# Crispy13/GeneFuseRust

Hardware: AMD Instinct MI355X
Metric: 150bp_reads_per_s_map_read_vs_druggable_shaped_index (higher is better)
Workload: dtype u32

## Files before the change

genefuserust_amd/csrc/gf_pipe_kernels.h:

```cpp
#pragma once

#include <hip/hip_runtime.h>

#include "../../include/gfmatch.h"
#include "gf_map_kernels.h"
#include "gf_table.h"

#ifndef GF_PROBE_NT
#define GF_PROBE_NT false
#endif

__device__ __forceinline__ uint32_t gf_spread16(uint32_t x) {
  x &= 0xFFFFu;
  x = (x | (x << 8)) & 0x00FF00FFu;
  x = (x | (x << 4)) & 0x0F0F0F0Fu;
  x = (x | (x << 2)) & 0x33333333u;
  x = (x | (x << 1)) & 0x55555555u;
  return x;
}

__device__ __forceinline__ uint32_t gf_gather_nibble_lsb(uint32_t x) {
  x &= 0x11111111u;
  x = (x | (x >> 3)) & 0x03030303u;
  x = (x | (x >> 6)) & 0x000F000Fu;
  x = (x | (x >> 12)) & 0xFFu;
  return x;
}

__device__ __forceinline__ unsigned int gf_wave_append(bool want, unsigned int* counter) {
  const uint64_t m = __ballot(want);
  unsigned int base = 0;
  if (m) {
    const int leader = __builtin_ctzll(m);
    if ((int)(threadIdx.x & 63) == leader) base = atomicAdd(counter, (unsigned int)__popcll(m));
    base = (unsigned int)__builtin_amdgcn_readlane((int)base, leader);
  }
  return base + (unsigned int)gf_lanes_below(m);
}

__device__ __forceinline__ unsigned int gf_wave_append_lds(bool want, unsigned int* s_counter) {
  const uint64_t m = __ballot(want);
  unsigned int base = 0;
  if (m) {
    const int leader = __builtin_ctzll(m);
    if ((int)(threadIdx.x & 63) == leader) base = atomicAdd(s_counter, (unsigned int)__popcll(m));
    base = (unsigned int)__builtin_amdgcn_readlane((int)base, leader);
  }
  return base + (unsigned int)gf_lanes_below(m);
}

#define GF_ENTRY_FILTERED 0x80000000u

template <int PW>
struct GfPipeEntryW {
  static constexpr int NT = PW <= 16 ? 4 : (PW + 3) / 4;
  static constexpr int EW = (2 + NT + PW + 3) / 4;
  uint32_t w[4 * EW];
};

template <int PW>
__device__ __forceinline__ void gf_entry_load(const GfPipeEntryW<PW>* e, uint32_t& r, uint32_t& v1v2,
                                              uint32_t (&m)[GfPipeEntryW<PW>::NT], uint32_t (&pk)[PW + 1]) {
  constexpr int NT = GfPipeEntryW<PW>::NT, EW = GfPipeEntryW<PW>::EW;
  uint32_t w[4 * EW];
  const gf_u32x4* src = (const gf_u32x4*)e;
#pragma unroll
  for (int j = 0; j < EW; ++j) {
#ifdef GF_ENTRY_NT
    const gf_u32x4 q = __builtin_nontemporal_load(src + j);
#else
    const gf_u32x4 q = src[j];
#endif
    w[4 * j] = q.x; w[4 * j + 1] = q.y; w[4 * j + 2] = q.z; w[4 * j + 3] = q.w;
  }
  r = w[0];
  v1v2 = w[1];
#pragma unroll
  for (int k = 0; k < NT; ++k) m[k] = w[2 + k];
#pragma unroll
  for (int j = 0; j < PW; ++j) pk[j] = w[2 + NT + j];
  pk[PW] = 0;
}

template <int PW>
__device__ __forceinline__ void gf_entry_store(GfPipeEntryW<PW>* e, uint32_t r, uint32_t v1v2,
                                               const uint32_t (&m)[GfPipeEntryW<PW>::NT], const uint32_t (&pk)[PW + 1]) {
  constexpr int NT = GfPipeEntryW<PW>::NT, EW = GfPipeEntryW<PW>::EW;
  uint32_t w[4 * EW];
  w[0] = r;
  w[1] = v1v2;
#pragma unroll
  for (int k = 0; k < NT; ++k) w[2 + k] = m[k];
#pragma unroll
  for (int j = 0; j < PW; ++j) w[2 + NT + j] = pk[j];
#pragma unroll
  for (int j = 2 + NT + PW; j < 4 * EW; ++j) w[j] = 0;
  gf_u32x4* dst = (gf_u32x4*)e;
#pragma unroll
  for (int j = 0; j < EW; ++j) {
    gf_u32x4 q;
    q.x = w[4 * j]; q.y = w[4 * j + 1]; q.z = w[4 * j + 2]; q.w = w[4 * j + 3];
#ifdef GF_ENTRY_NT
    __builtin_nontemporal_store(q, dst + j);
#else
    dst[j] = q;
#endif
  }
}

__device__ __forceinline__ uint32_t gf_cut_pk(const uint32_t* s_pk, uint32_t w0, uint32_t sh, int j) {
  return __builtin_amdgcn_alignbit(s_pk[w0 + j + 1], s_pk[w0 + j], sh);
}

__device__ __forceinline__ uint32_t gf_cut_iv(const uint32_t* s_iv, uint32_t pos, int L, int j) {
  const uint32_t bp = pos + 16u * (uint32_t)j;
  uint32_t b = __builtin_amdgcn_alignbit(s_iv[(bp >> 5) + 1], s_iv[bp >> 5], bp & 31u) & 0xFFFFu;
  const int k = L - 16 * j;
  if (k < 16) b |= k <= 0 ? 0xFFFFu : ((0xFFFFu << k) & 0xFFFFu);
  return gf_spread16(b);
}

__device__ __forceinline__ uint32_t gf_clean16(uint32_t z_lo, uint32_t z_hi) {
  uint32_t lo = ~z_lo & 0x55555555u, hi = ~z_hi & 0x55555555u;
#pragma unroll
  for (uint32_t sh = 2; sh <= 16; sh <<= 1) {
    lo &= __builtin_amdgcn_alignbit(hi, lo, sh);
    hi &= hi >> sh;
  }
  return lo;
}

__device__ __forceinline__ void gf_convert16(const uint4& q, uint32_t& code32, uint32_t& bad16) {
  const uint32_t z0 = q.x & 0x06060606u, z1 = q.y & 0x06060606u, z2 = q.z & 0x06060606u, z3 = q.w & 0x06060606u;
  const uint32_t d0 = q.x ^ __builtin_amdgcn_perm(0x00470054u, 0x00430041u, z0), d1 = q.y ^ __builtin_amdgcn_perm(0x00470054u, 0x00430041u, z1);
  const uint32_t d2 = q.z ^ __builtin_amdgcn_perm(0x00470054u, 0x00430041u, z2), d3 = q.w ^ __builtin_amdgcn_perm(0x00470054u, 0x00430041u, z3);
  const uint32_t e0 = __builtin_amdgcn_udot4(z0, 0x40100401u, 0u, false), e1 = __builtin_amdgcn_udot4(z1, 0x40100401u, 0u, false);
  const uint32_t e2 = __builtin_amdgcn_udot4(z2, 0x40100401u, 0u, false), e3 = __builtin_amdgcn_udot4(z3, 0x40100401u, 0u, false);
  code32 = ((e0 + (e1 << 8) + (e2 << 16)) >> 1) | ((e3 >> 1) << 24);
  bad16 = 0;
  if (d0 | d1 | d2 | d3) {
    const uint32_t n0 = (((d0 & 0x7F7F7F7Fu) + 0x7F7F7F7Fu) | d0) & 0x80808080u;
    const uint32_t n1 = (((d1 & 0x7F7F7F7Fu) + 0x7F7F7F7Fu) | d1) & 0x80808080u;
    const uint32_t n2 = (((d2 & 0x7F7F7F7Fu) + 0x7F7F7F7Fu) | d2) & 0x80808080u;
    const uint32_t n3 = (((d3 & 0x7F7F7F7Fu) + 0x7F7F7F7Fu) | d3) & 0x80808080u;
    bad16 = (((n0 >> 7) * 0x00204081u) >> 21 & 0xFu) | ((((n1 >> 7) * 0x00204081u) >> 21 & 0xFu) << 4) |
            ((((n2 >> 7) * 0x00204081u) >> 21 & 0xFu) << 8) | ((((n3 >> 7) * 0x00204081u) >> 21 & 0xFu) << 12);
  }
}

__device__ __forceinline__ uint32_t gf_window_mask(int nwin, int k) {
  const int m = nwin - 32 * k;
  return m >= 32 ? 0xFFFFFFFFu : (m <= 0 ? 0u : ((1u << m) - 1u));
}

#ifndef GF_SEED_FILTER_MASK
#define GF_SEED_FILTER_MASK 2u
#endif
#ifndef GF_MID_SEEDS
#define GF_MID_SEEDS 2
#endif
#ifndef GF_FILTER_AUX
#define GF_FILTER_AUX 0
#endif
#ifndef GF_SVS_WAVES_PER_SIMD
#define GF_SVS_WAVES_PER_SIMD 4
#endif
#ifndef GF_FQ_CAP
#define GF_FQ_CAP 96
#endif

template <int PW>
__device__ __forceinline__ int gf_filter_queue_pass(const GfTable& T, gf_u32x4* s_q, int q_len, int lane,
                                                    uint8_t* __restrict__ counts, GfPipeEntryW<PW>* my_list,
                                                    unsigned int* s_cnt) {
  static_assert(PW == 10, "the queue holds the 64-byte entries of reads of up to 160 bases");
  constexpr int NT = GfPipeEntryW<PW>::NT;
  const int m = q_len < 64 ? q_len : 64;
  const int base = q_len - m;
  const bool act = lane < m;
  uint32_t w[16];
#pragma unroll
  for (int j = 0; j < 16; ++j) w[j] = 0;
  if (act) {
#pragma unroll
    for (int j = 0; j < 4; ++j) {
      const gf_u32x4 q = s_q[(base + lane) * 4 + j];
      w[4 * j] = q.x; w[4 * j + 1] = q.y; w[4 * j + 2] = q.z; w[4 * j + 3] = q.w;
    }
  }
  gf_wave_lds_sync();
  const __amdgpu_buffer_rsrc_t filter_rsrc =
      __builtin_amdgcn_make_buffer_rsrc((void*)T.bloom, 0, (int)(T.bloom_words * 4u), 0x00020000);
  const uint32_t filter_bytes = T.bloom_words * 4u;
  const uint32_t rnd = w[1];
  bool alive = false;
  if (act) {
    uint32_t wlo = w[2 + NT];
#pragma unroll
    for (int j = 0; j < PW; ++j) {
      const uint32_t whi = j + 1 < PW ? w[2 + NT + j + 1] : 0u;
      const uint32_t byte = (w[2 + (j >> 2)] >> (8 * (j & 3))) & 0xFFu;
      uint32_t word[2], bits[2];
#pragma unroll
      for (int t = 0; t < 2; ++t) {
        const uint32_t s14 = __builtin_amdgcn_alignbit(whi, wlo, 16u * (uint32_t)t + 8u * rnd + 4u) & 0x0FFFFFFFu;
        const uint32_t h2 = GF_BLOOM_HASH((s14));
        bits[t] = GF_BLOOM_BITS(h2);
        const uint32_t nb = (byte & (3u << (4 * t + 2 * rnd))) ? filter_bytes : 0u;
        word[t] = __builtin_amdgcn_raw_buffer_load_b32(filter_rsrc, __umulhi(h2, nb) & ~3u, 0, GF_FILTER_AUX);
      }
      uint32_t fail2 = 0;
#pragma unroll
      for (int t = 0; t < 2; ++t) {
        const uint32_t d = bits[t] & ~word[t];
        uint32_t f;
        asm("v_min_u32 %0, %1, 1" : "=v"(f) : "v"(d));
        fail2 |= f << (4 * t);
      }
      fail2 <<= 2 * rnd;
      w[2 + (j >> 2)] &= ~((fail2 | (fail2 << 1)) << (8 * (j & 3)));
      wlo = whi;
    }
    uint32_t x[NT];
#pragma unroll
    for (int k = 0; k < NT; ++k) x[k] = (w[2 + k] | (w[2 + k] >> 1)) & 0x55555555u;
    alive = gf_vote_bound_pairs<4 * PW - 3>(x) >= GF_MAJOR_KEYS / 2;
  }
  if (act && !alive) counts[w[0]] = 0;
  const bool again = act && alive && rnd == 0u;
  const uint64_t am = __ballot(again);
  if (again) {
    const int slot = base + gf_lanes_below(am);
    w[1] = 1u;
#pragma unroll
    for (int j = 0; j < 4; ++j) {
      gf_u32x4 q;
      q.x = w[4 * j]; q.y = w[4 * j + 1]; q.z = w[4 * j + 2]; q.w = w[4 * j + 3];
      s_q[slot * 4 + j] = q;
    }
  }
  const bool emit = act && alive && rnd != 0u;
  const unsigned int slot_b = gf_wave_append_lds(emit, s_cnt);
  if (emit) {
    w[1] = GF_ENTRY_FILTERED;
    gf_u32x4* dst = (gf_u32x4*)(my_list + slot_b);
#pragma unroll
    for (int j = 0; j < 4; ++j) {
      gf_u32x4 q;
      q.x = w[4 * j]; q.y = w[4 * j + 1]; q.z = w[4 * j + 2]; q.w = w[4 * j + 3];
      dst[j] = q;
    }
  }
  gf_wave_lds_sync();
  return base + __popcll(am);
}

template <int PW>
__device__ __forceinline__ void gf_verify_words2(const GfTable& T, const uint32_t* pk, uint32_t K,
                                                 uint32_t (&vmb)[GfPipeEntryW<PW>::NT], uint32_t (&hmb)[GfPipeEntryW<PW>::NT]) {
  constexpr int NT = GfPipeEntryW<PW>::NT;
#pragma unroll
  for (int k = 0; k < NT; ++k) vmb[k] = hmb[k] = 0;
  const uint2* gp = (const uint2*)T.gdu + (K >> 4);
  if (PW == 10 && T.gdt != nullptr) {
    const uint32_t p = K >> 4, t = __umulhi(p, 0xAAAAAAABu) >> 2;
    gp = (const uint2*)T.gdt + 16u * t + (p - 6u * t);
  }
  const uint32_t bo = 2u * (K & 15u);
  uint2 gw[PW + 1];
#pragma unroll
  for (int j = 0; j < PW + 1; ++j) gw[j] = gp[j];
  uint32_t zz_cur;
  {
    const uint32_t x = pk[0] ^ __builtin_amdgcn_alignbit(gw[1].x, gw[0].x, bo);
    zz_cur = (x | (x >> 1)) & 0x55555555u;
  }
#pragma unroll
  for (int j = 0; j < PW; ++j) {
    uint32_t zz_next = 0x55555555u;
    if (j + 1 < PW) {
      const uint32_t x = pk[j + 1] ^ __builtin_amdgcn_alignbit(gw[j + 2 <= PW ? j + 2 : PW].x, gw[j + 1].x, bo);
      zz_next = (x | (x >> 1)) & 0x55555555u;
    }
    const uint32_t u = __builtin_amdgcn_alignbit(gw[j + 1].y, gw[j].y, bo);
    const uint32_t clean = gf_clean16(zz_cur, zz_next);
    vmb[j >> 2] |= gf_gather_nibble_lsb(clean & u & 0x11111111u) << (8 * (j & 3));
    hmb[j >> 2] |= gf_gather_nibble_lsb(clean & (u >> 1) & 0x11111111u) << (8 * (j & 3));
    zz_cur = zz_next;
  }
}

template <int PW>
__device__ __forceinline__ int gf_high_queue_pass(const GfTable& T, gf_u32x4* s_q, int q_back, int lane,
                                                  uint8_t* __restrict__ counts, GfPipeEntryW<PW>* my_list,
                                                  unsigned int* s_cnt) {
  static_assert(PW == 10, "the queue holds the 64-byte entries of reads of up to 160 bases");
  constexpr int NT = GfPipeEntryW<PW>::NT;
  const int m = q_back < 64 ? q_back : 64;
  const int base = GF_FQ_CAP - q_back;
  const bool act = lane < m;
  uint32_t w[16];
#pragma unroll
  for (int j = 0; j < 16; ++j) w[j] = 0;
  if (act) {
#pragma unroll
    for (int j = 0; j < 4; ++j) {
      const gf_u32x4 q = s_q[(base + lane) * 4 + j];
      w[4 * j] = q.x; w[4 * j + 1] = q.y; w[4 * j + 2] = q.z; w[4 * j + 3] = q.w;
    }
  }
  bool emit = false;
  if (act) {
    uint32_t vk[NT], hk[NT];
    gf_verify_words2<PW>(T, &w[2 + NT], w[1], vk, hk);
    int v1 = 0, h = 0, nvalid = 0;
#pragma unroll
    for (int k = 0; k < NT; ++k) {
      const uint32_t cw = w[2 + k];
      vk[k] &= cw;
      hk[k] &= cw & ~vk[k];
      v1 += __popc(vk[k]);
      h += __popc(hk[k]);
      nvalid += __popc(cw);
      w[2 + k] = cw & ~vk[k] & ~hk[k];
    }
    const int open = nvalid - v1 - h;
    if (v1 + open < GF_MAJOR_KEYS / 2 || open < GF_MINOR_KEYS / 2) counts[w[0]] = 0;
    else emit = true;
    w[1] = v1 > 0 ? (uint32_t)v1 : GF_ENTRY_FILTERED;
  }
  const unsigned int slot_b = gf_wave_append_lds(emit, s_cnt);
  if (emit) {
    gf_u32x4* dst = (gf_u32x4*)(my_list + slot_b);
#pragma unroll
    for (int j = 0; j < 4; ++j) {
      gf_u32x4 q;
      q.x = w[4 * j]; q.y = w[4 * j + 1]; q.z = w[4 * j + 2]; q.w = w[4 * j + 3];
      dst[j] = q;
    }
  }
  gf_wave_lds_sync();
  return q_back - m;
}

template <int PW, bool PACKED = false>
__global__ __launch_bounds__(256, PW <= 10 ? GF_SVS_WAVES_PER_SIMD : 4) void gf_k_seedverify_stream(
    GfTable T, const uint8_t* __restrict__ bases, const uint32_t* __restrict__ g_pk,
    const uint16_t* __restrict__ g_iv, const int64_t* __restrict__ offsets, int64_t n, int lmax,
    int batch_max, uint8_t* __restrict__ counts, GfPipeEntryW<PW>* __restrict__ list_b,
    unsigned int* __restrict__ blk_cnt, int64_t per_block, uint32_t* __restrict__ list_long,
    unsigned int* __restrict__ ctr) {
  constexpr int TILE_BYTES = 64 * 16 * PW;
  constexpr int TILE_CHUNKS = TILE_BYTES / 16 + 1;
  constexpr int PK_WORDS = (TILE_CHUNKS + PW + 2 + 3) & ~3;
  constexpr int IV_WORDS = (TILE_CHUNKS + PW + 2) / 2 + 2;
  constexpr int NLOAD = (TILE_CHUNKS + 63) / 64;
  constexpr int IW = (PW + 1) / 2;
  constexpr int NT = GfPipeEntryW<PW>::NT;
  __shared__ __attribute__((aligned(16))) uint32_t s_pk_all[4][PK_WORDS];
  __shared__ uint32_t s_iv_all[4][IV_WORDS];
#ifndef GF_SV_INLINE_ROUNDS
  constexpr bool QUEUED = PW == 10;
#else
  constexpr bool QUEUED = false;
#endif
  __shared__ gf_u32x4 s_q_all[QUEUED ? 4 : 1][QUEUED ? GF_FQ_CAP * 4 : 1];
  __shared__ unsigned int s_cnt;
  if (threadIdx.x == 0) s_cnt = 0;
  __syncthreads();
  const int lane = threadIdx.x & 63;
  const int wave = __builtin_amdgcn_readfirstlane((int)(threadIdx.x >> 6));
  uint32_t* s_pk = s_pk_all[wave];
  uint32_t* s_iv = s_iv_all[wave];
  gf_u32x4* s_q = s_q_all[QUEUED ? wave : 0];
  int q_len = 0;
  int q_back = 0;
  const int64_t r_lo = (int64_t)blockIdx.x * per_block;
  int64_t n_lim = n;
  if (T.n_dev) {
    const int64_t nd = *T.n_dev;
    n_lim = nd < n ? (nd < 0 ? 0 : nd) : n;
  }
  const int64_t r_hi = r_lo + per_block < n_lim ? r_lo + per_block : n_lim;
  const int64_t fixed_len = T.fixed_len;
  GfPipeEntryW<PW>* my_list = list_b + r_lo;
  for (int64_t g0 = r_lo + 64 * (int64_t)wave; g0 < r_hi; g0 += 256) {
    const int64_t g1 = g0 + 64 < r_hi ? g0 + 64 : r_hi;
    int64_t r0 = g0;
    while (r0 < g1) {
#define GF_OFF(x) (fixed_len ? (int64_t)(x) * fixed_len : offsets[x])
      const int64_t base_off = GF_OFF(r0);
      const uint8_t* p0 = bases + base_off;
      const uint32_t mis = PACKED ? (uint32_t)(base_off & 15) : (uint32_t)((uintptr_t)p0 & 15u);
      const uint4* src = (const uint4*)(p0 - mis);
      const int64_t c0 = base_off >> 4;
      const int64_t r = r0 + lane;
      int64_t off0 = 0, off1 = 0;
      if (r < g1) {
        off0 = GF_OFF(r);
        off1 = GF_OFF(r + 1);
      }
      const bool fits = r < g1 && (uint64_t)(off1 - base_off) + mis <= (uint64_t)TILE_BYTES;
      int nfit = __popcll(__ballot(fits));
      const bool oversize = nfit == 0;
      if (oversize) nfit = 1;
      gf_wave_lds_sync();
      const uint32_t chunks = oversize ? 0u : (uint32_t)((GF_OFF(r0 + nfit) - base_off) + mis + 15) >> 4;
      if (PACKED && chunks > 0) {
        uint32_t qp[NLOAD], qi[NLOAD];
#pragma unroll
        for (int k = 0; k < NLOAD; ++k) {
          const uint32_t c = (uint32_t)lane + 64u * (uint32_t)k;
          const int64_t cc = c0 + (int64_t)(c < chunks ? c : chunks - 1);
          qp[k] = __builtin_nontemporal_load(g_pk + cc);
          qi[k] = __builtin_nontemporal_load(g_iv + cc);
        }
#pragma unroll
        for (int k = 0; k < NLOAD; ++k) {
          const uint32_t c = (uint32_t)lane + 64u * (uint32_t)k;
          if (c < chunks) {
            s_pk[c] = qp[k];
            ((uint16_t*)s_iv)[c] = (uint16_t)qi[k];
          }
        }
      } else if (chunks > 0) {
        uint4 q[NLOAD];
#pragma unroll
        for (int k = 0; k < NLOAD; ++k) {
          const uint32_t c = (uint32_t)lane + 64u * (uint32_t)k;
#if defined(GF_STAGE_AUX)
          const __amdgpu_buffer_rsrc_t stage_rsrc = __builtin_amdgcn_make_buffer_rsrc((void*)src, 0, (int)(chunks * 16u), 0x00020000);
          const auto t = __builtin_amdgcn_raw_buffer_load_b128(stage_rsrc, 16u * (c < chunks ? c : chunks - 1), 0, GF_STAGE_AUX);
          q[k] = make_uint4(t[0], t[1], t[2], t[3]);
#elif !defined(GF_STAGE_TEMPORAL)
          const gf_u32x4 t = __builtin_nontemporal_load((const gf_u32x4*)(src + (c < chunks ? c : chunks - 1)));
          q[k] = make_uint4(t.x, t.y, t.z, t.w);
#else
          q[k] = src[c < chunks ? c : chunks - 1];
#endif
        }
#pragma unroll
        for (int k = 0; k < NLOAD; ++k) {
          const uint32_t c = (uint32_t)lane + 64u * (uint32_t)k;
          uint32_t code32, bad16;
          gf_convert16(q[k], code32, bad16);
          if (c < chunks) {
            s_pk[c] = code32;
            ((uint16_t*)s_iv)[c] = (uint16_t)bad16;
          }
        }
      }
      gf_wave_lds_sync();
      __builtin_amdgcn_sched_barrier(0);
      const bool in_range = lane < nfit;
      bool undecided = false, long1k = false, long4k = false;
      bool queued = false;
      bool hqueued = false;
      uint32_t K_q = 0;
      uint32_t pp_q[NT];
#pragma unroll
      for (int k = 0; k < NT; ++k) pp_q[k] = 0;
      uint32_t e_v1v2 = 0, e_todo[NT];
#pragma unroll
      for (int k = 0; k < NT; ++k) e_todo[k] = 0;
      uint32_t w0 = 0, sh = 0;
#if defined(GF_ABLATE_SV) && GF_ABLATE_SV == 6
      if (in_range) counts[r] = s_pk[((uint32_t)(off0 - base_off) + mis) >> 4] == 0x1234567u ? 1 : 0;
      if (false) {
#else
      if (in_range) {
#endif
        const int64_t len64 = off1 - off0;
        if (T.skip != nullptr && T.skip[r] > 0) {
          counts[r] = 0;
        } else if (len64 > batch_max) {
          counts[r] = GF_COUNT_TOO_LONG;
        } else if (len64 > lmax) {
          long1k = len64 <= 1024;
          long4k = !long1k;
        } else if (len64 < GF_KMER + 2 * (GF_MAJOR_KEYS / 2 - 1)) {
          counts[r] = 0;
        } else {
          const int L = (int)len64;
          const uint32_t pos = (uint32_t)(off0 - base_off) + mis;
          w0 = pos >> 4;
          sh = 2u * (pos & 15u);
          uint32_t anybad = 0;
          {
            const uint32_t v0 = pos >> 5, vs = pos & 31u;
            uint32_t lo = s_iv[v0];
#pragma unroll
            for (int j = 0; j < IW; ++j) {
              const uint32_t hi = s_iv[v0 + j + 1];
              uint32_t b = __builtin_amdgcn_alignbit(hi, lo, vs);
              const int k = L - 32 * j;
              if (k < 32) b &= k <= 0 ? 0u : ((1u << k) - 1u);
              anybad |= b;
              lo = hi;
            }
          }
          uint32_t cwb[NT];
          int nvalid;
          uint32_t key[4];
          uint32_t okm = 0;
#pragma unroll
          for (int s = 0; s < 4; ++s) key[s] = 2 * s < PW ? gf_cut_pk(s_pk, w0, sh, 2 * s) : 0u;
          if (!anybad) {
            nvalid = (L - GF_KMER) / 2 + 1;
#pragma unroll
            for (int k = 0; k < NT; ++k) cwb[k] = gf_window_mask(nvalid, k);
#pragma unroll
            for (int s = 0; s < 4; ++s) okm |= (2 * s < PW && 16 * s < nvalid ? 1u : 0u) << s;
          } else {
#pragma unroll
            for (int k = 0; k < NT; ++k) cwb[k] = 0;
            nvalid = 0;
            uint32_t z_cur = gf_cut_iv(s_iv, pos, L, 0);
#pragma unroll
            for (int j = 0; j < PW; ++j) {
              const uint32_t z_next = j + 1 < PW ? gf_cut_iv(s_iv, pos, L, j + 1) : 0x55555555u;
              const uint32_t cw = gf_clean16(z_cur, z_next) & 0x11111111u;
              nvalid += __popc(cw);
              cwb[j >> 2] |= gf_gather_nibble_lsb(cw) << (8 * (j & 3));
              if ((j & 1) == 0 && j < 8) okm |= (cw & 1u) << (j >> 1);
              z_cur = z_next;
            }
          }
#if defined(GF_ABLATE_SV) && GF_ABLATE_SV == 1
          if ((nvalid ^ key[0] ^ key[1] ^ key[2] ^ key[3] ^ cwb[0] ^ cwb[1] ^ cwb[2] ^ cwb[NT - 1] ^ okm) == 0x1234567u) counts[r] = 1;
          okm = 0;
#endif
#if defined(GF_ABLATE_SV) && GF_ABLATE_SV == 5
          if ((nvalid ^ key[0] ^ key[1] ^ key[2] ^ key[3] ^ cwb[0] ^ cwb[1] ^ cwb[2] ^ cwb[NT - 1] ^ okm) == 0x1234567u) counts[r] = 1;
          okm = 0;
          nvalid = 0;
#pragma unroll
          for (int k = 0; k < NT; ++k) cwb[k] = 0;
#endif
          uint32_t kill[2] = {0, 0};
          uint32_t khigh[2] = {0, 0};
          uint32_t K = GF_NONE_LIN;
          uint32_t Krep = GF_NONE_LIN;
          if (T.bloom_in_l2 & GF_SEED_FILTER_MASK) {
            const uint32_t h2 = GF_BLOOM_HASH((key[0] >> 4));
            const uint32_t fb = GF_BLOOM_BITS(h2);
            if ((T.bloom[GF_BLOOM_WORD(h2, T.bloom_words)] & fb) != fb) {
              okm &= ~1u;
              kill[0] |= 3u;
            }
          }
          if (okm & 1u) {
            okm &= ~1u;
            const uint32_t val = gf_lookup(T, key[0]);
            const uint32_t ty = val >> GF_TYPE_SHIFT;
            if (ty == GF_TYPE_UNIQUE) K = val & GF_LIN_MASK;
            else if (ty != GF_TYPE_DUPES) {
              kill[0] |= 1u;
              if (ty == GF_TYPE_HIGH) {
                khigh[0] |= 1u;
                if ((val & GF_LIN_MASK) != GF_LIN_MASK) Krep = val & GF_LIN_MASK;
              }
            }
          }
          if (K == GF_NONE_LIN && (T.bloom_in_l2 & GF_SEED_FILTER_MASK)) {
            uint32_t fw[4], fb[4];
#pragma unroll
            for (int s = 1; s < 4; ++s) {
              const uint32_t h2 = GF_BLOOM_HASH((key[s] >> 4));
              fb[s] = GF_BLOOM_BITS(h2);
              fw[s] = T.bloom[GF_BLOOM_WORD(h2, T.bloom_words)];
            }
#pragma unroll
            for (int s = 1; s < 4; ++s)
              if (2 * s < PW && (fw[s] & fb[s]) != fb[s]) {
                okm &= ~(1u << s);
                kill[s >> 1] |= 3u << (16 * (s & 1));
              }
          }
#if defined(GF_ABLATE_SV) && GF_ABLATE_SV == 3
          if (okm == 0x1234567u) counts[r] = 1;
          okm = 0;
#endif
          if (T.bloom_in_l2 != 2) okm &= (1u << GF_MID_SEEDS) - 1u;
          while (okm != 0 && K == GF_NONE_LIN) {
            const int s = __builtin_ctz(okm);
            okm &= okm - 1;
            const uint32_t ks = s == 0 ? key[0] : (s == 1 ? key[1] : (s == 2 ? key[2] : key[3]));
            const uint32_t val = gf_lookup(T, ks);
            const uint32_t ty = val >> GF_TYPE_SHIFT;
            if (ty == GF_TYPE_UNIQUE) K = (val & GF_LIN_MASK) - 32u * (uint32_t)s;
            else if (ty != GF_TYPE_DUPES) {
              kill[s >> 1] |= 1u << (16 * (s & 1));
              if (ty == GF_TYPE_HIGH) {
                khigh[s >> 1] |= 1u << (16 * (s & 1));
                if (Krep == GF_NONE_LIN && (val & GF_LIN_MASK) != GF_LIN_MASK) Krep = (val & GF_LIN_MASK) - 32u * (uint32_t)s;
              }
            }
          }
          nvalid -= __popc(cwb[0] & kill[0]) + __popc(cwb[1] & kill[1]);
          cwb[0] &= ~kill[0];
          cwb[1] &= ~kill[1];
#if defined(GF_ABLATE_SV) && GF_ABLATE_SV == 4
          if (K == 0x1234567u) counts[r] = 1;
          K = GF_NONE_LIN;
#endif
          bool filt_done = false, filt_dead = false;
#ifdef GF_ABLATE_EXTRA_VALU
          uint32_t ablate_sink = 0;
#endif
          const __amdgpu_buffer_rsrc_t filter_rsrc =
              __builtin_amdgcn_make_buffer_rsrc((void*)T.bloom, 0, (int)(T.bloom_words * 4u), 0x00020000);
          const uint32_t filter_bytes = T.bloom_words * 4u;
          uint32_t pp[NT];
#pragma unroll
          for (int k = 0; k < NT; ++k) pp[k] = 0;
#ifndef GF_SV_NO_INLINE_FILTER
#ifndef GF_FILTER_ALLPAIRS
          if (QUEUED && K == GF_NONE_LIN && T.bloom_in_l2 == 2) {
            filt_done = true;
            if (nvalid < GF_MAJOR_KEYS / 2) {
              filt_dead = true;
            } else if ((khigh[0] | khigh[1]) && Krep != GF_NONE_LIN) {
              hqueued = true;
#pragma unroll
              for (int k = 0; k < NT; ++k) pp_q[k] = cwb[k];
              K_q = Krep;
            } else if (khigh[0] | khigh[1]) {
#pragma unroll
              for (int k = 0; k < NT; ++k) pp[k] = cwb[k];
              pp[0] |= khigh[0];
              pp[1] |= khigh[1];
            } else {
              queued = true;
#pragma unroll
              for (int k = 0; k < NT; ++k) pp_q[k] = cwb[k];
              pp_q[0] |= khigh[0];
              pp_q[1] |= khigh[1];
            }
          } else if (PW == 10 && K == GF_NONE_LIN && T.bloom_in_l2 == 2) {
            filt_done = true;
#pragma unroll
            for (int k = 0; k < NT; ++k) pp[k] = cwb[k];
            pp[0] |= khigh[0];
            pp[1] |= khigh[1];
            bool alive = true;
#pragma unroll 1
            for (uint32_t rnd = 0; rnd < 2; ++rnd) {
              if (alive) {
                uint32_t wlo = gf_cut_pk(s_pk, w0, sh, 0);
#pragma unroll
                for (int j = 0; j < PW; ++j) {
                  const uint32_t whi = j + 1 < PW ? gf_cut_pk(s_pk, w0, sh, j + 1) : 0u;
                  const uint32_t byte = (pp[j >> 2] >> (8 * (j & 3))) & 0xFFu;
                  uint32_t word[2], bits[2];
#pragma unroll
                  for (int t = 0; t < 2; ++t) {
                    const uint32_t s14 = __builtin_amdgcn_alignbit(whi, wlo, 16u * (uint32_t)t + 8u * rnd + 4u) & 0x0FFFFFFFu;
                    const uint32_t h2 = GF_BLOOM_HASH((s14));
#ifdef GF_ABLATE_EXTRA_VALU
                    ablate_sink ^= gf_canon14(s14 ^ 0x05A5A5A5u);
#endif
                    bits[t] = GF_BLOOM_BITS(h2);
                    const uint32_t nb = (byte & (3u << (4 * t + 2 * rnd))) ? filter_bytes : 0u;
                    word[t] = __builtin_amdgcn_raw_buffer_load_b32(filter_rsrc, __umulhi(h2, nb) & ~3u, 0, GF_FILTER_AUX);
                  }
                  uint32_t fail2 = 0;
#pragma unroll
                  for (int t = 0; t < 2; ++t) {
                    const uint32_t d = bits[t] & ~word[t];
                    uint32_t f;
                    asm("v_min_u32 %0, %1, 1" : "=v"(f) : "v"(d));
                    fail2 |= f << (4 * t);
                  }
                  fail2 <<= 2 * rnd;
                  pp[j >> 2] &= ~((fail2 | (fail2 << 1)) << (8 * (j & 3)));
                  wlo = whi;
                }
                uint32_t x[NT];
#pragma unroll
                for (int k = 0; k < NT; ++k) x[k] = (pp[k] | (pp[k] >> 1)) & 0x55555555u;
                alive = gf_vote_bound_pairs<4 * PW - 3>(x) >= GF_MAJOR_KEYS / 2;
              }
            }
            filt_dead = !alive;
          } else
#endif
          if (K == GF_NONE_LIN && T.bloom_in_l2 == 2) {
            filt_done = true;
            int npos = 0, rem = nvalid;
            uint32_t wlo = gf_cut_pk(s_pk, w0, sh, 0);
#pragma unroll
            for (int j = 0; j < PW; ++j) {
              const uint32_t whi = j + 1 < PW ? gf_cut_pk(s_pk, w0, sh, j + 1) : 0u;
#ifndef GF_FILTER_OLD
              if (!filt_dead) {
                const uint32_t byte = (cwb[j >> 2] >> (8 * (j & 3))) & 0xFFu;
                uint32_t word[4], bits[4];
#pragma unroll
                for (int u = 0; u < 4; ++u) {
                  const uint32_t s14 = __builtin_amdgcn_alignbit(whi, wlo, 8u * (uint32_t)u + 4u) & 0x0FFFFFFFu;
                  const uint32_t h2 = GF_BLOOM_HASH((s14));
                  bits[u] = GF_BLOOM_BITS(h2);
                  const uint32_t nb = (byte & (3u << (2 * u))) ? filter_bytes : 0u;
                  word[u] = __builtin_amdgcn_raw_buffer_load_b32(filter_rsrc, __umulhi(h2, nb) & ~3u, 0, GF_FILTER_AUX);
                }
                uint32_t fail2 = 0;
#pragma unroll
                for (int u = 0; u < 4; ++u) {
                  const uint32_t t = bits[u] & ~word[u];
                  uint32_t f;
                  asm("v_min_u32 %0, %1, 1" : "=v"(f) : "v"(t));
                  fail2 |= f << (2 * u);
                }
                const uint32_t pbyte = byte & ~(fail2 | (fail2 << 1));
                pp[j >> 2] |= pbyte << (8 * (j & 3));
                npos += __popc(pbyte);
                rem -= __popc(byte);
                filt_dead = npos + rem < GF_MAJOR_KEYS / 2;
              }
#else
              if (!filt_dead) {
                const uint32_t byte = (cwb[j >> 2] >> (8 * (j & 3))) & 0xFFu;
                uint32_t word[4], bits[4], both[4];
#pragma unroll
                for (int u = 0; u < 4; ++u) {
                  both[u] = (byte >> (2 * u)) & 3u;
                  const uint32_t s14 = __builtin_amdgcn_alignbit(whi, wlo, 8u * (uint32_t)u + 4u) & 0x0FFFFFFFu;
                  const uint32_t h2 = GF_BLOOM_HASH((s14));
                  bits[u] = GF_BLOOM_BITS(h2);
                  word[u] = 0;
                  if (both[u]) word[u] = T.bloom[GF_BLOOM_WORD(h2, T.bloom_words)];
                }
#pragma unroll
                for (int u = 0; u < 4; ++u) {
                  const int cnt = (int)(both[u] & 1u) + (int)(both[u] >> 1);
                  rem -= cnt;
                  if (both[u] && (word[u] & bits[u]) == bits[u]) {
                    pp[j >> 2] |= both[u] << (8 * (j & 3) + 2 * u);
                    npos += cnt;
                  }
                }
                filt_dead = npos + rem < GF_MAJOR_KEYS / 2;
              }
#endif
              wlo = whi;
            }
          }
#endif
          uint32_t vmb[NT];
#pragma unroll
          for (int k = 0; k < NT; ++k) vmb[k] = 0;
          if (K != GF_NONE_LIN) {
            const uint2* gp = (const uint2*)T.gdu + (K >> 4);
            if (PW == 10 && T.gdt != nullptr) {
              const uint32_t p = K >> 4, t = __umulhi(p, 0xAAAAAAABu) >> 2;
              gp = (const uint2*)T.gdt + 16u * t + (p - 6u * t);
            }
            const uint32_t bo = 2u * (K & 15u);
            uint2 gw[PW + 1];
#pragma unroll
            for (int j = 0; j < PW + 1; ++j) gw[j] = gp[j];
            uint32_t zz_cur;
            {
              const uint32_t x = gf_cut_pk(s_pk, w0, sh, 0) ^ __builtin_amdgcn_alignbit(gw[1].x, gw[0].x, bo);
              zz_cur = (x | (x >> 1)) & 0x55555555u;
              if (anybad) zz_cur |= gf_cut_iv(s_iv, pos, L, 0);
            }
#pragma unroll
            for (int j = 0; j < PW; ++j) {
              uint32_t zz_next = 0x55555555u;
              if (j + 1 < PW) {
                const uint32_t x = gf_cut_pk(s_pk, w0, sh, j + 1) ^
                                   __builtin_amdgcn_alignbit(gw[j + 2 <= PW ? j + 2 : PW].x, gw[j + 1].x, bo);
                zz_next = (x | (x >> 1)) & 0x55555555u;
                if (anybad) zz_next |= gf_cut_iv(s_iv, pos, L, j + 1);
              }
              const uint32_t u = __builtin_amdgcn_alignbit(gw[j + 1].y, gw[j].y, bo);
              const uint32_t ver = gf_clean16(zz_cur, zz_next) & u & 0x11111111u;
              vmb[j >> 2] |= gf_gather_nibble_lsb(ver) << (8 * (j & 3));
              zz_cur = zz_next;
              if (j & 1) __builtin_amdgcn_sched_barrier(0);
            }
          }
          int v1 = 0;
#ifdef GF_ABLATE_EXTRA_VALU
          if (ablate_sink == 0x12345u) v1 = 1;
#endif
#pragma unroll
          for (int k = 0; k < NT; ++k) {
            vmb[k] &= cwb[k];
            v1 += __popc(vmb[k]);
          }
          const int open = nvalid - v1;
          if (queued || hqueued) {
          } else if (v1 + open < GF_MAJOR_KEYS / 2 || open < GF_MINOR_KEYS / 2 || filt_dead) {
            counts[r] = 0;
          } else if (filt_done) {
            undecided = true;
            e_v1v2 = GF_ENTRY_FILTERED;
#pragma unroll
            for (int k = 0; k < NT; ++k) e_todo[k] = pp[k];
          } else if (QUEUED && K != GF_NONE_LIN && (khigh[0] | khigh[1])) {
            hqueued = true;
            K_q = K;
#pragma unroll
            for (int k = 0; k < NT; ++k) pp_q[k] = cwb[k];
          } else {
            undecided = true;
            e_v1v2 = (uint32_t)v1;
#pragma unroll
            for (int k = 0; k < NT; ++k) e_todo[k] = cwb[k] & ~vmb[k];
            if (v1 == 0) {
              e_todo[0] |= khigh[0];
              e_todo[1] |= khigh[1];
            }
          }
        }
      }
      __builtin_amdgcn_sched_barrier(0);
      if constexpr (QUEUED) {
        const uint64_t qm = __ballot(queued), hm = __ballot(hqueued);
        if (qm | hm) {
          const int n_new = __popcll(qm), n_newh = __popcll(hm);
          while (q_len + q_back + n_new + n_newh > GF_FQ_CAP) {
            if (q_len >= q_back) q_len = gf_filter_queue_pass<PW>(T, s_q, q_len, lane, counts, my_list, &s_cnt);
            else q_back = gf_high_queue_pass<PW>(T, s_q, q_back, lane, counts, my_list, &s_cnt);
          }
          if (queued || hqueued) {
            const int slot = queued ? q_len + gf_lanes_below(qm) : GF_FQ_CAP - 1 - q_back - gf_lanes_below(hm);
            uint32_t ew[16];
            ew[0] = (uint32_t)r;
            ew[1] = queued ? 0u : K_q;
#pragma unroll
            for (int k = 0; k < NT; ++k) ew[2 + k] = pp_q[k];
#pragma unroll
            for (int j = 0; j < PW; ++j) ew[2 + NT + j] = gf_cut_pk(s_pk, w0, sh, j);
#pragma unroll
            for (int j = 0; j < 4; ++j) {
              gf_u32x4 q;
              q.x = ew[4 * j]; q.y = ew[4 * j + 1]; q.z = ew[4 * j + 2]; q.w = ew[4 * j + 3];
              s_q[slot * 4 + j] = q;
            }
          }
          q_len += n_new;
          q_back += n_newh;
          gf_wave_lds_sync();
        }
      }
      const unsigned int slot_b = gf_wave_append_lds(undecided, &s_cnt);
#ifdef GF_ENTRY_DIRECT_STORE
      constexpr bool direct_store = true;
#else
      constexpr bool direct_store = PW > 16;
#endif
      if constexpr (direct_store) {
        if (undecided) {
          uint32_t pkw[PW + 1];
#pragma unroll
          for (int j = 0; j < PW; ++j) pkw[j] = gf_cut_pk(s_pk, w0, sh, j);
          pkw[PW] = 0;
          gf_entry_store<PW>(my_list + slot_b, (uint32_t)r, e_v1v2, e_todo, pkw);
        }
      } else {
      const uint64_t um = __ballot(undecided);
      if (um) {
        constexpr int EW = GfPipeEntryW<PW>::EW;
        constexpr int CH = PK_WORDS / (4 * EW);
        const int cnt = __popcll(um), rank = gf_lanes_below(um);
        const unsigned int base =
            (unsigned int)__builtin_amdgcn_readlane((int)(slot_b - (unsigned int)rank), __builtin_ctzll(um));
        uint32_t ew[4 * EW];
#pragma unroll
        for (int j = 0; j < 4 * EW; ++j) ew[j] = 0;
        if (undecided) {
          ew[0] = (uint32_t)r;
          ew[1] = e_v1v2;
#pragma unroll
          for (int k = 0; k < NT; ++k) ew[2 + k] = e_todo[k];
#pragma unroll
          for (int j = 0; j < PW; ++j) ew[2 + NT + j] = gf_cut_pk(s_pk, w0, sh, j);
        }
        uint4* s_ent = (uint4*)s_pk;
        for (int c0 = 0; c0 < cnt; c0 += CH) {
          gf_wave_lds_sync();
          if (undecided && rank >= c0 && rank < c0 + CH) {
#pragma unroll
            for (int j = 0; j < EW; ++j)
              s_ent[(rank - c0) * EW + j] = make_uint4(ew[4 * j], ew[4 * j + 1], ew[4 * j + 2], ew[4 * j + 3]);
          }
          gf_wave_lds_sync();
          const int nvec = (cnt - c0 < CH ? cnt - c0 : CH) * EW;
          uint4* dst = (uint4*)(my_list + base + c0);
          for (int k = lane; k < nvec; k += 64) dst[k] = s_ent[k];
        }
      }
      }
      if constexpr (QUEUED) {
        while (q_len >= 64) q_len = gf_filter_queue_pass<PW>(T, s_q, q_len, lane, counts, my_list, &s_cnt);
        while (q_back >= 64) q_back = gf_high_queue_pass<PW>(T, s_q, q_back, lane, counts, my_list, &s_cnt);
      }
      if (batch_max > lmax) {
        const unsigned int s1 = gf_wave_append(long1k, ctr + 2);
        if (long1k) list_long[s1] = (uint32_t)r;
        const unsigned int s4 = gf_wave_append(long4k, ctr + 3);
        if (long4k) list_long[n - 1 - (int64_t)s4] = (uint32_t)r;
      }
      r0 += nfit;
    }
  }
  if constexpr (QUEUED) {
    while (q_len > 0) q_len = gf_filter_queue_pass<PW>(T, s_q, q_len, lane, counts, my_list, &s_cnt);
    while (q_back > 0) q_back = gf_high_queue_pass<PW>(T, s_q, q_back, lane, counts, my_list, &s_cnt);
  }
  __syncthreads();
  if (threadIdx.x == 0) blk_cnt[blockIdx.x] = s_cnt;
}

template <int PW>
__device__ __forceinline__ void gf_entries_to_lds(gf_u32x4* s_ent, const GfPipeEntryW<PW>* chunk, unsigned int cnt) {
  constexpr int EW = GfPipeEntryW<PW>::EW, EWP = EW + 1;
  const gf_u32x4* src = (const gf_u32x4*)chunk;
#pragma unroll
  for (int k = 0; k < EW; ++k) {
    const unsigned int g = (unsigned int)k * 256u + threadIdx.x;
    if (g < cnt * EW) s_ent[(g / EW) * EWP + g % EW] = src[g];
  }
}
template <int PW>
__device__ __forceinline__ void gf_entry_from_lds(const gf_u32x4* s_ent, uint32_t& r, uint32_t& v1v2,
                                                  uint32_t (&m)[GfPipeEntryW<PW>::NT], uint32_t (&pk)[PW + 1],
                                                  unsigned int e = 0xFFFFFFFFu) {
  constexpr int NT = GfPipeEntryW<PW>::NT, EW = GfPipeEntryW<PW>::EW, EWP = EW + 1;
  if (e == 0xFFFFFFFFu) e = threadIdx.x;
  uint32_t w[4 * EW];
#pragma unroll
  for (int j = 0; j < EW; ++j) {
    const gf_u32x4 q = s_ent[e * EWP + j];
    w[4 * j] = q.x; w[4 * j + 1] = q.y; w[4 * j + 2] = q.z; w[4 * j + 3] = q.w;
  }
  r = w[0];
  v1v2 = w[1];
#pragma unroll
  for (int k = 0; k < NT; ++k) m[k] = w[2 + k];
#pragma unroll
  for (int j = 0; j < PW; ++j) pk[j] = w[2 + NT + j];
  pk[PW] = 0;
}

template <int PW>
__global__ __launch_bounds__(256) void gf_k_probe_filter(GfTable T, GfPipeEntryW<PW>* __restrict__ list_b,
                                                         const unsigned int* __restrict__ blk_cnt, int64_t per_block,
                                                         uint8_t* __restrict__ counts,
                                                         unsigned int* __restrict__ blk_cnt2, int phase, int nparts) {
  constexpr int EW = GfPipeEntryW<PW>::EW, EWP = EW + 1;
  __shared__ gf_u32x4 s_ent[256 * EWP];
  __shared__ unsigned short s_perm[256];
  __shared__ unsigned int s_kind[2][4];
  __shared__ unsigned int s_cnt;
  if (threadIdx.x == 0) s_cnt = 0;
  __syncthreads();
  const unsigned int nb = blk_cnt[blockIdx.x];
  const uint32_t part_words = (T.bloom_words + (uint32_t)nparts - 1) / (uint32_t)nparts;
  const uint32_t part_lo = (uint32_t)phase * part_words, part_hi = part_lo + part_words;
  const bool last_part = phase == nparts - 1;
  GfPipeEntryW<PW>* my_list = list_b + (int64_t)blockIdx.x * per_block;
  for (unsigned int t0 = 0; t0 < nb; t0 += 256) {
    const unsigned int t = t0 + threadIdx.x;
    const unsigned int cnt = nb - t0 < 256u ? nb - t0 : 256u;
    gf_entries_to_lds<PW>(s_ent, my_list + t0, cnt);
    s_perm[threadIdx.x] = 0xFFFFu;
    __syncthreads();
    {
      const int lane = threadIdx.x & 63, wv = threadIdx.x >> 6;
      bool with_cand = false;
      if (t < nb) {
        const gf_u32x4 q0 = s_ent[threadIdx.x * EWP];
        const uint32_t h = q0.y;
        with_cand = (h & GF_ENTRY_FILTERED) == 0 && T.bloom_words != 0 && !(PW == 10 && (h & 0xFFFFu) == 0);
      }
      const uint64_t mc = __ballot(with_cand), mn = __ballot(t < nb && !with_cand);
      if (lane == 0) {
        s_kind[0][wv] = (unsigned int)__popcll(mn);
        s_kind[1][wv] = (unsigned int)__popcll(mc);
      }
      __syncthreads();
      unsigned int before_n = 0, before_c = 0;
      for (int k = 0; k < wv; ++k) {
        before_n += s_kind[0][k];
        before_c += s_kind[1][k];
      }
      if (t < nb) {
        const unsigned int pos = with_cand ? 255u - (before_c + (unsigned int)gf_lanes_below(mc))
                                           : before_n + (unsigned int)gf_lanes_below(mn);
        s_perm[pos] = (unsigned short)threadIdx.x;
      }
      __syncthreads();
    }
    const unsigned int ent = s_perm[threadIdx.x];
    bool alive = false;
    constexpr int NT = GfPipeEntryW<PW>::NT;
    uint32_t r = 0, v1v2 = 0, m[NT], pk[PW + 1];
    uint32_t pp[NT];
#pragma unroll
    for (int k = 0; k < NT; ++k) m[k] = pp[k] = 0;
    if (ent != 0xFFFFu) {
      gf_entry_from_lds<PW>(s_ent, r, v1v2, m, pk, ent);
      const bool filtered = (v1v2 & GF_ENTRY_FILTERED) != 0;
      const int v1 = (int)(v1v2 & 0xFFu), v2 = (int)((v1v2 >> 8) & 0xFFu);
      const bool no_candidate = PW == 10 && !filtered && v1 == 0 && v2 == 0 && T.bloom_words != 0;
      bool dead = false;
      if (filtered) {
#pragma unroll
        for (int k = 0; k < NT; ++k) pp[k] = m[k];
      } else if (no_candidate) {
        auto ask = [&](uint32_t par) {
#pragma unroll
          for (int j = 0; j < PW; ++j) {
            const uint32_t byte = (m[j >> 2] >> (8 * (j & 3))) & 0xFFu;
            uint32_t word[2], bits[2];
#pragma unroll
            for (int u2 = 0; u2 < 2; ++u2) {
              const uint32_t s14 = __builtin_amdgcn_alignbit(pk[j + 1], pk[j], 16u * (uint32_t)u2 + 8u * par + 4u) & 0x0FFFFFFFu;
              const uint32_t h2 = GF_BLOOM_HASH((s14));
              bits[u2] = GF_BLOOM_BITS(h2);
              const uint32_t widx = GF_BLOOM_WORD(h2, T.bloom_words);
              const bool mine = widx >= part_lo && widx < part_hi && (byte & (3u << (4 * u2 + 2 * par))) != 0;
              word[u2] = 0xFFFFFFFFu;
              if (mine) word[u2] = T.bloom[widx];
            }
            uint32_t fail2 = 0;
#pragma unroll
            for (int u2 = 0; u2 < 2; ++u2) fail2 |= ((bits[u2] & ~word[u2]) != 0 ? 1u : 0u) << (4 * u2);
            fail2 <<= 2 * par;
            m[j >> 2] &= ~((fail2 | (fail2 << 1)) << (8 * (j & 3)));
          }
        };
        auto bound = [&]() {
          uint32_t x[NT];
#pragma unroll
          for (int k = 0; k < NT; ++k) x[k] = (m[k] | (m[k] >> 1)) & 0x55555555u;
          return gf_vote_bound_pairs<4 * PW - 3>(x);
        };
        if (nparts == 1) {
          ask(0u);
          dead = bound() < GF_MAJOR_KEYS / 2;
          if (!dead) {
            ask(1u);
            dead = bound() < GF_MAJOR_KEYS / 2;
          }
          v1v2 |= GF_ENTRY_FILTERED;
        } else if (!last_part) {
          ask(0u);
          ask(1u);
        } else {
          ask(0u);
          dead = bound() < GF_MAJOR_KEYS / 2;
          if (!dead) {
            ask(1u);
            dead = bound() < GF_MAJOR_KEYS / 2;
          }
          v1v2 |= GF_ENTRY_FILTERED;
        }
#pragma unroll
        for (int k = 0; k < NT; ++k) pp[k] = m[k];
      } else if (T.bloom_words) {
        int npos = 0, rem = 0;
#pragma unroll
        for (int k = 0; k < NT; ++k) rem += __popc(m[k]);
#pragma unroll
        for (int q0 = 0; q0 < 4 * PW; q0 += 4) {
          if (!dead) {
            uint32_t word[4], bits[4], both[4];
#pragma unroll
            for (int u = 0; u < 4; ++u) {
              const int q = q0 + u;
              const int wbit = (2 * q) & 31, wword = (2 * q) >> 5;
              both[u] = wword < NT ? (m[wword] >> wbit) & 3u : 0u;
              const int b0 = 4 * q + 2;
              const int j = b0 >> 4;
              const uint32_t sh14 = 2u * (uint32_t)(b0 & 15);
              const uint32_t s14 = __builtin_amdgcn_alignbit(pk[j + 1], pk[j], sh14) & 0x0FFFFFFFu;
              const uint32_t h2 = GF_BLOOM_HASH((s14));
              bits[u] = GF_BLOOM_BITS(h2);
              const uint32_t widx = GF_BLOOM_WORD(h2, T.bloom_words);
              const bool mine = widx >= part_lo && widx < part_hi;
              word[u] = mine ? 0u : bits[u];
              if (both[u] && mine) word[u] = T.bloom[widx];
            }
#pragma unroll
            for (int u = 0; u < 4; ++u) {
              const int q = q0 + u;
              const int cnt = (int)(both[u] & 1u) + (int)(both[u] >> 1);
              rem -= cnt;
              if (both[u] && (word[u] & bits[u]) == bits[u]) {
                pp[(2 * q) >> 5 < NT ? (2 * q) >> 5 : 0] |= both[u] << ((2 * q) & 31);
                npos += cnt;
              }
            }
            dead = (v1 + npos + rem < GF_MAJOR_KEYS / 2) || (v2 + npos + rem < GF_MINOR_KEYS / 2);
          }
        }
        if (last_part) v1v2 |= GF_ENTRY_FILTERED;
      } else {
#pragma unroll
        for (int k = 0; k < NT; ++k) pp[k] = m[k];
        int left = 0;
#pragma unroll
        for (int k = 0; k < NT; ++k) left += __popc(m[k]);
        dead = !filtered && ((v1 + left < GF_MAJOR_KEYS / 2) || (v2 + left < GF_MINOR_KEYS / 2));
      }
      if (dead) counts[r] = 0;
      alive = !dead;
    }
    const unsigned int base = s_cnt;
    __syncthreads();
    const unsigned int slot = gf_wave_append_lds(alive, &s_cnt);
    if (alive) {
      uint32_t w[4 * EW];
      w[0] = r;
      w[1] = v1v2;
#pragma unroll
      for (int k = 0; k < NT; ++k) w[2 + k] = pp[k];
#pragma unroll
      for (int j = 0; j < PW; ++j) w[2 + NT + j] = pk[j];
#pragma unroll
      for (int j = 2 + NT + PW; j < 4 * EW; ++j) w[j] = 0;
#pragma unroll
      for (int j = 0; j < EW; ++j) {
        gf_u32x4 q;
        q.x = w[4 * j]; q.y = w[4 * j + 1]; q.z = w[4 * j + 2]; q.w = w[4 * j + 3];
        s_ent[(slot - base) * EWP + j] = q;
      }
    }
    __syncthreads();
    {
      const unsigned int n_alive = s_cnt - base;
      gf_u32x4* dst = (gf_u32x4*)(my_list + base);
#pragma unroll
      for (int k = 0; k < EW; ++k) {
        const unsigned int g = (unsigned int)k * 256u + threadIdx.x;
        if (g < n_alive * EW) dst[g] = s_ent[(g / EW) * EWP + g % EW];
      }
    }
    __syncthreads();
  }
  if (threadIdx.x == 0) blk_cnt2[blockIdx.x] = s_cnt;
}

template <int PW, bool HIGHBIT = false>
__device__ __forceinline__ void gf_verify_words(const GfTable& T, const uint32_t (&pk)[PW + 1], uint32_t K,
                                                uint32_t (&vmb)[GfPipeEntryW<PW>::NT]) {
  constexpr int NT = GfPipeEntryW<PW>::NT;
#pragma unroll
  for (int k = 0; k < NT; ++k) vmb[k] = 0;
  const uint2* gp = (const uint2*)T.gdu + (K >> 4);
  const uint32_t bo = 2u * (K & 15u);
  uint2 gw[PW + 1];
#pragma unroll
  for (int j = 0; j < PW + 1; ++j) gw[j] = gp[j];
  uint32_t zz_cur;
  {
    const uint32_t x = pk[0] ^ __builtin_amdgcn_alignbit(gw[1].x, gw[0].x, bo);
    zz_cur = (x | (x >> 1)) & 0x55555555u;
  }
#pragma unroll
  for (int j = 0; j < PW; ++j) {
    uint32_t zz_next = 0x55555555u;
    if (j + 1 < PW) {
      const uint32_t x = pk[j + 1] ^ __builtin_amdgcn_alignbit(gw[j + 2 <= PW ? j + 2 : PW].x, gw[j + 1].x, bo);
      zz_next = (x | (x >> 1)) & 0x55555555u;
    }
    uint32_t u = __builtin_amdgcn_alignbit(gw[j + 1].y, gw[j].y, bo);
    if (HIGHBIT) u >>= 1;
    const uint32_t ver = gf_clean16(zz_cur, zz_next) & u & 0x11111111u;
    vmb[j >> 2] |= gf_gather_nibble_lsb(ver) << (8 * (j & 3));
    zz_cur = zz_next;
  }
}

template <int PW>
__global__ __launch_bounds__(256) void gf_k_probe_buckets(GfTable T, const GfPipeEntryW<PW>* __restrict__ list_b,
                                                          const unsigned int* __restrict__ blk_cnt2,
                                                          int64_t per_block, uint8_t* __restrict__ counts,
// ... 167 lines not shown
```

Baseline: 9.498 billion.

## Hold packed read words in registers and chain clean-window computation backwards

For 10-word reads, the packed read words are cut from LDS once into registers and reused by key extraction, filtering, verification and entry stores, instead of being re-cut from LDS at each use. The verify loops now run backwards, using a rolling 4-word chain that carries the partially reduced mask between words, so each word's clean mask is no longer recomputed from scratch. The nibble gather is replaced with a udot4 instruction. This trades more live registers, with possible occupancy pressure, for fewer LDS reads and ALU ops.

```diff
diff --git a/genefuserust_amd/csrc/gf_pipe_kernels.h b/genefuserust_amd/csrc/gf_pipe_kernels.h
--- a/genefuserust_amd/csrc/gf_pipe_kernels.h
+++ b/genefuserust_amd/csrc/gf_pipe_kernels.h
@@ -22,9 +22,7 @@
 __device__ __forceinline__ uint32_t gf_gather_nibble_lsb(uint32_t x) {
   x &= 0x11111111u;
   x = (x | (x >> 3)) & 0x03030303u;
-  x = (x | (x >> 6)) & 0x000F000Fu;
-  x = (x | (x >> 12)) & 0xFFu;
-  return x;
+  return __builtin_amdgcn_udot4(x, 0x40100401u, 0u, false);
 }
 
 __device__ __forceinline__ unsigned int gf_wave_append(bool want, unsigned int* counter) {
@@ -128,6 +126,17 @@
     hi &= hi >> sh;
   }
   return lo;
+}
+
+__device__ __forceinline__ uint32_t gf_clean16_chain(uint32_t z, uint32_t (&n)[4]) {
+  uint32_t l = ~z & 0x55555555u;
+#pragma unroll
+  for (int k = 0; k < 4; ++k) {
+    const uint32_t t = l & __builtin_amdgcn_alignbit(n[k], l, 2u << k);
+    n[k] = l;
+    l = t;
+  }
+  return l;
 }
 
 __device__ __forceinline__ void gf_convert16(const uint4& q, uint32_t& code32, uint32_t& bad16) {
@@ -270,23 +279,15 @@
   uint2 gw[PW + 1];
 #pragma unroll
   for (int j = 0; j < PW + 1; ++j) gw[j] = gp[j];
-  uint32_t zz_cur;
-  {
-    const uint32_t x = pk[0] ^ __builtin_amdgcn_alignbit(gw[1].x, gw[0].x, bo);
-    zz_cur = (x | (x >> 1)) & 0x55555555u;
-  }
-#pragma unroll
-  for (int j = 0; j < PW; ++j) {
-    uint32_t zz_next = 0x55555555u;
-    if (j + 1 < PW) {
-      const uint32_t x = pk[j + 1] ^ __builtin_amdgcn_alignbit(gw[j + 2 <= PW ? j + 2 : PW].x, gw[j + 1].x, bo);
-      zz_next = (x | (x >> 1)) & 0x55555555u;
-    }
+  uint32_t run[4] = {0, 0, 0, 0};
+#pragma unroll
+  for (int j = PW - 1; j >= 0; --j) {
+    const uint32_t x = pk[j] ^ __builtin_amdgcn_alignbit(gw[j + 1].x, gw[j].x, bo);
+    const uint32_t zz = (x | (x >> 1)) & 0x55555555u;
     const uint32_t u = __builtin_amdgcn_alignbit(gw[j + 1].y, gw[j].y, bo);
-    const uint32_t clean = gf_clean16(zz_cur, zz_next);
+    const uint32_t clean = gf_clean16_chain(zz, run);
     vmb[j >> 2] |= gf_gather_nibble_lsb(clean & u & 0x11111111u) << (8 * (j & 3));
     hmb[j >> 2] |= gf_gather_nibble_lsb(clean & (u >> 1) & 0x11111111u) << (8 * (j & 3));
-    zz_cur = zz_next;
   }
 }
 
@@ -464,6 +465,14 @@
 #pragma unroll
       for (int k = 0; k < NT; ++k) e_todo[k] = 0;
       uint32_t w0 = 0, sh = 0;
+      constexpr bool HOLD = PW == 10;
+      uint32_t pk_held[HOLD ? PW : 1];
+#pragma unroll
+      for (int j = 0; j < (HOLD ? PW : 1); ++j) pk_held[j] = 0;
+      auto pk_word = [&](int j) -> uint32_t {
+        if constexpr (HOLD) return pk_held[j];
+        else return gf_cut_pk(s_pk, w0, sh, j);
+      };
 #if defined(GF_ABLATE_SV) && GF_ABLATE_SV == 6
       if (in_range) counts[r] = s_pk[((uint32_t)(off0 - base_off) + mis) >> 4] == 0x1234567u ? 1 : 0;
       if (false) {
@@ -485,6 +494,15 @@
           const uint32_t pos = (uint32_t)(off0 - base_off) + mis;
           w0 = pos >> 4;
           sh = 2u * (pos & 15u);
+          if constexpr (HOLD) {
+            uint32_t lo = s_pk[w0];
+#pragma unroll
+            for (int j = 0; j < PW; ++j) {
+              const uint32_t hi = s_pk[w0 + j + 1];
+              pk_held[j] = __builtin_amdgcn_alignbit(hi, lo, sh);
+              lo = hi;
+            }
+          }
           uint32_t anybad = 0;
           {
             const uint32_t v0 = pos >> 5, vs = pos & 31u;
@@ -504,7 +522,7 @@
           uint32_t key[4];
           uint32_t okm = 0;
 #pragma unroll
-          for (int s = 0; s < 4; ++s) key[s] = 2 * s < PW ? gf_cut_pk(s_pk, w0, sh, 2 * s) : 0u;
+          for (int s = 0; s < 4; ++s) key[s] = 2 * s < PW ? pk_word(2 * s) : 0u;
           if (!anybad) {
             nvalid = (L - GF_KMER) / 2 + 1;
 #pragma unroll
@@ -647,10 +665,10 @@
 #pragma unroll 1
             for (uint32_t rnd = 0; rnd < 2; ++rnd) {
               if (alive) {
-                uint32_t wlo = gf_cut_pk(s_pk, w0, sh, 0);
+                uint32_t wlo = pk_word(0);
 #pragma unroll
                 for (int j = 0; j < PW; ++j) {
-                  const uint32_t whi = j + 1 < PW ? gf_cut_pk(s_pk, w0, sh, j + 1) : 0u;
+                  const uint32_t whi = j + 1 < PW ? pk_word(j + 1) : 0u;
                   const uint32_t byte = (pp[j >> 2] >> (8 * (j & 3))) & 0xFFu;
                   uint32_t word[2], bits[2];
 #pragma unroll
@@ -688,10 +706,10 @@
           if (K == GF_NONE_LIN && T.bloom_in_l2 == 2) {
             filt_done = true;
             int npos = 0, rem = nvalid;
-            uint32_t wlo = gf_cut_pk(s_pk, w0, sh, 0);
+            uint32_t wlo = pk_word(0);
 #pragma unroll
             for (int j = 0; j < PW; ++j) {
-              const uint32_t whi = j + 1 < PW ? gf_cut_pk(s_pk, w0, sh, j + 1) : 0u;
+              const uint32_t whi = j + 1 < PW ? pk_word(j + 1) : 0u;
 #ifndef GF_FILTER_OLD
               if (!filt_dead) {
                 const uint32_t byte = (cwb[j >> 2] >> (8 * (j & 3))) & 0xFFu;
@@ -760,26 +778,16 @@
             uint2 gw[PW + 1];
 #pragma unroll
             for (int j = 0; j < PW + 1; ++j) gw[j] = gp[j];
-            uint32_t zz_cur;
-            {
-              const uint32_t x = gf_cut_pk(s_pk, w0, sh, 0) ^ __builtin_amdgcn_alignbit(gw[1].x, gw[0].x, bo);
-              zz_cur = (x | (x >> 1)) & 0x55555555u;
-              if (anybad) zz_cur |= gf_cut_iv(s_iv, pos, L, 0);
-            }
-#pragma unroll
-            for (int j = 0; j < PW; ++j) {
-              uint32_t zz_next = 0x55555555u;
-              if (j + 1 < PW) {
-                const uint32_t x = gf_cut_pk(s_pk, w0, sh, j + 1) ^
-                                   __builtin_amdgcn_alignbit(gw[j + 2 <= PW ? j + 2 : PW].x, gw[j + 1].x, bo);
-                zz_next = (x | (x >> 1)) & 0x55555555u;
-                if (anybad) zz_next |= gf_cut_iv(s_iv, pos, L, j + 1);
-              }
+            uint32_t run[4] = {0, 0, 0, 0};
+#pragma unroll
+            for (int j = PW - 1; j >= 0; --j) {
+              const uint32_t x = pk_word(j) ^ __builtin_amdgcn_alignbit(gw[j + 1].x, gw[j].x, bo);
+              uint32_t zz = (x | (x >> 1)) & 0x55555555u;
+              if (anybad) zz |= gf_cut_iv(s_iv, pos, L, j);
               const uint32_t u = __builtin_amdgcn_alignbit(gw[j + 1].y, gw[j].y, bo);
-              const uint32_t ver = gf_clean16(zz_cur, zz_next) & u & 0x11111111u;
+              const uint32_t ver = gf_clean16_chain(zz, run) & u & 0x11111111u;
               vmb[j >> 2] |= gf_gather_nibble_lsb(ver) << (8 * (j & 3));
-              zz_cur = zz_next;
-              if (j & 1) __builtin_amdgcn_sched_barrier(0);
+              if (!(j & 1)) __builtin_amdgcn_sched_barrier(0);
             }
           }
           int v1 = 0;
@@ -834,7 +842,7 @@
 #pragma unroll
             for (int k = 0; k < NT; ++k) ew[2 + k] = pp_q[k];
 #pragma unroll
-            for (int j = 0; j < PW; ++j) ew[2 + NT + j] = gf_cut_pk(s_pk, w0, sh, j);
+            for (int j = 0; j < PW; ++j) ew[2 + NT + j] = pk_word(j);
 #pragma unroll
             for (int j = 0; j < 4; ++j) {
               gf_u32x4 q;
@@ -857,7 +865,7 @@
         if (undecided) {
           uint32_t pkw[PW + 1];
 #pragma unroll
-          for (int j = 0; j < PW; ++j) pkw[j] = gf_cut_pk(s_pk, w0, sh, j);
+          for (int j = 0; j < PW; ++j) pkw[j] = pk_word(j);
           pkw[PW] = 0;
           gf_entry_store<PW>(my_list + slot_b, (uint32_t)r, e_v1v2, e_todo, pkw);
         }
@@ -878,7 +886,7 @@
 #pragma unroll
           for (int k = 0; k < NT; ++k) ew[2 + k] = e_todo[k];
 #pragma unroll
-          for (int j = 0; j < PW; ++j) ew[2 + NT + j] = gf_cut_pk(s_pk, w0, sh, j);
+          for (int j = 0; j < PW; ++j) ew[2 + NT + j] = pk_word(j);
         }
         uint4* s_ent = (uint4*)s_pk;
         for (int c0 = 0; c0 < cnt; c0 += CH) {
```

Measured after the change: 9.606 billion, median of 6. 1.01x the previous value.
